# yukw777/EILEV

Measured on AMD Instinct MI355X. Metric: clips/sec (8-frame, 16 in-context) encode+generate, eilev-blip2-opt-2.7b, higher is better.
Workload: dtype bf16

## Files before the change

### eilev_amd/csrc/gemm_common.h

```cpp
#pragma once
#include "common.h"
#ifndef EILEV_ST_AUX
#define EILEV_ST_AUX 2
#endif
#include <type_traits>
#include <utility>

namespace {


constexpr int BK = 64;

__device__ __forceinline__ int swz(int row, int c) { return (c ^ ((row >> 1) & 7)) << 4; }

template <class F, int... I>
__device__ __forceinline__ void static_for_impl(F &&f, std::integer_sequence<int, I...>) {
    (f(std::integral_constant<int, I>{}), ...);
}
template <int N, class F>
__device__ __forceinline__ void static_for(F &&f) {
    static_for_impl(f, std::make_integer_sequence<int, N>{});
}

__device__ __forceinline__ void tile_coords(const GemmArgs &g, int tiles_m, int tiles_n, int &tm, int &tn, int t = blockIdx.x) {
    const int nwg = tiles_m * tiles_n;
    const int xcd = t & 7, q = nwg >> 3, r = nwg & 7;
    t = (xcd < r ? xcd * (q + 1) : r * (q + 1) + (xcd - r) * q) + (t >> 3);
    if (g.dbg & DBG_GEMM_ROW_MAJOR_TILES) {
        tm = t / tiles_n;
        tn = t % tiles_n;
        return;
    }
    const int gsel = (g.dbg >> DBG_GEMM_GROUP_SHIFT) & 3;
    const int GROUP_M = gsel == 1 ? 4 : gsel == 2 ? 8 : gsel == 3 ? 16 : (tiles_n <= 8 ? 4 : 8);
    const int width = GROUP_M * tiles_n, group = t / width, first = group * GROUP_M;
    const int gsz = min(tiles_m - first, GROUP_M), in = t - group * width;
    tm = first + in % gsz;
    tn = in / gsz;
}

template <int WM, int WN, int EPI, int IBEG = 0, int IEND = WM / 32, int LN = 0, bool FASTG = false>
__device__ __forceinline__ void gemm_epilogue(const GemmArgs &g, f32x16 (&acc)[WM / 32][WN / 32], char *smem, int m0, int n0,
                                              int wm, int wn, int wid, int lane) {
    constexpr int TN = WN / 32;
    constexpr int RS = WN * 2 + 8;
    constexpr int ROWS = (IEND - IBEG) * 32;
    const int l31 = lane & 31, hi = lane >> 5;
    const int wrow0 = m0 + wm * WM, wcol0 = n0 + wn * WN;
    if (g.out_f32) {
#pragma unroll
        for (int i = IBEG; i < IEND; ++i) {
            const int row = wrow0 + i * 32 + l31;
#pragma unroll
            for (int j = 0; j < TN; ++j)
#pragma unroll
                for (int q = 0; q < 4; ++q) {
                    const int col = wcol0 + j * 32 + q * 8 + hi * 4;
                    if (row < g.M && col < g.N && !((g.dbg & DBG_GEMM_ROW0_STORES) && row > 0)) {
                        float *dst = reinterpret_cast<float *>(g.C) + (int64_t)row * g.ldc + col;
#pragma unroll
                        for (int e = 0; e < 4; ++e) {
                            float v = acc[i][j][q * 4 + e];
                            if (g.ascale) v *= g.ascale[row];
                            if (g.wscale && col + e < g.N) v *= g.wscale[col + e];
                            if (g.bias) v += (float)g.bias[col + e];
                            if (col + e < g.scale_cols) v *= g.scale;
                            if (EPI == 1) v = gelu_erf(v);
                            else if (EPI == 2) v = fmaxf(v, 0.0f);
                            if (g.resid) v += (float)g.resid[(int64_t)row * g.ldr + col + e];
                            if (col + e < g.N) {
                                if (g.k_slice > 0) atomicAdd(dst + e, v);
                                else dst[e] = v;
                            }
                        }
                    }
                }
        }
        return;
    }
    if (g.dbg & DBG_GEMM_NO_EPILOGUE) {
        float keep = 0.0f;
#pragma unroll
        for (int i = IBEG; i < IEND; ++i)
#pragma unroll
            for (int j = 0; j < TN; ++j) keep += acc[i][j][0] + acc[i][j][7] + acc[i][j][15];
        if (keep == 123.456f) reinterpret_cast<float *>(g.C)[0] = keep;
        return;
    }
    float st1[LN == 2 ? IEND - IBEG : 1], st2[LN == 2 ? IEND - IBEG : 1];
    if constexpr (LN == 2) {
#pragma unroll
        for (int i = 0; i < IEND - IBEG; ++i) st1[i] = st2[i] = 0.0f;
    }
    char *reg = smem + wid * (ROWS * RS);
    const int wrow1 = wrow0 + IBEG * 32;
    const int srow = lane >> 3, schunk = lane & 7;
    const bool patch = g.patch_group > 0;
    const bool interior = wrow1 + ROWS <= g.M && wcol0 + WN <= g.N && !patch && !(g.dbg & DBG_GEMM_ROW0_STORES);
    const bool has_res = g.resid != nullptr;
    const bool has_scale = g.scale_cols > 0;
    if (has_res) {
        if (interior) {
            const bf16 *rp = g.resid + (int64_t)(wrow1 + srow) * g.ldr + wcol0 + schunk * 8;
            char *dp = reg + srow * RS + schunk * 16;
#pragma unroll 4
            for (int it = 0; it < ROWS / 8; ++it) {
                const bf16x8 v = *reinterpret_cast<const bf16x8 *>(rp);
                bf16x4 *d = reinterpret_cast<bf16x4 *>(dp);
                d[0] = (bf16x4){v[0], v[1], v[2], v[3]};
                d[1] = (bf16x4){v[4], v[5], v[6], v[7]};
                rp += 8 * g.ldr;
                dp += 8 * RS;
            }
        } else {
#pragma unroll 2
            for (int it = 0; it < ROWS / 8; ++it) {
                const int lr = it * 8 + srow, row = wrow1 + lr, col = wcol0 + schunk * 8;
                bf16x8 v = zero8();
                if (row < g.M && col < g.N) {
                    const int64_t rrow = patch ? 1 + (row % g.patch_group) : row;
                    v = *reinterpret_cast<const bf16x8 *>(g.resid + rrow * g.ldr + col);
                }
                bf16x4 *d = reinterpret_cast<bf16x4 *>(reg + lr * RS + schunk * 16);
                d[0] = (bf16x4){v[0], v[1], v[2], v[3]};
                d[1] = (bf16x4){v[4], v[5], v[6], v[7]};
            }
        }
    }
#pragma unroll
    for (int j = 0; j < TN; ++j) {
#pragma unroll
        for (int q = 0; q < 4; ++q) {
            const int lc = j * 32 + q * 8 + hi * 4, col = wcol0 + lc;
            float bv[4] = {0.f, 0.f, 0.f, 0.f};
            if (g.bias && col < g.N) {
                const bf16x4 b4 = *reinterpret_cast<const bf16x4 *>(g.bias + col);
#pragma unroll
                for (int e = 0; e < 4; ++e) bv[e] = (float)b4[e];
            }
            float sc[4] = {1.f, 1.f, 1.f, 1.f};
            if (has_scale) {
#pragma unroll
                for (int e = 0; e < 4; ++e) sc[e] = (col + e) < g.scale_cols ? g.scale : 1.0f;
            }
            char *cp = reg + l31 * RS + lc * 2;
            constexpr int NI = IEND - IBEG;
            float v[NI][4];
            if (g.wscale) {
#pragma unroll
                for (int e = 0; e < 4; ++e) {
                    const float ws = col + e < g.N ? g.wscale[col + e] : 1.0f;
#pragma unroll
                    for (int i = 0; i < NI; ++i) acc[IBEG + i][j][q * 4 + e] *= ws;
                }
            }
            if (g.ascale) {
#pragma unroll
                for (int i = 0; i < NI; ++i) {
                    const int row = wrow0 + (IBEG + i) * 32 + l31;
                    const float as = row < g.M ? g.ascale[row] : 1.0f;
#pragma unroll
                    for (int e = 0; e < 4; ++e) acc[IBEG + i][j][q * 4 + e] *= as;
                }
            }
            if (LN == 1) {
#pragma unroll
                for (int i = 0; i < NI; ++i) {
                    const int row = wrow0 + (IBEG + i) * 32 + l31;
                    const float la = row < g.M ? g.ln_rows[2 * (int64_t)row] : 1.0f;
#pragma unroll
                    for (int e = 0; e < 4; ++e) acc[IBEG + i][j][q * 4 + e] *= la;
                }
            }
#pragma unroll
            for (int i = 0; i < NI; ++i)
#pragma unroll
                for (int e = 0; e < 4; ++e) {
                    v[i][e] = acc[IBEG + i][j][q * 4 + e] + bv[e];
                    if (has_scale) v[i][e] *= sc[e];
                    if (EPI == 2) v[i][e] = fmaxf(v[i][e], 0.0f);
                }
            if (EPI == 1) {
                f32x2 x[2 * NI];
#pragma unroll
                for (int i = 0; i < NI; ++i) {
                    x[2 * i] = (f32x2){v[i][0], v[i][1]};
                    x[2 * i + 1] = (f32x2){v[i][2], v[i][3]};
                }
                if constexpr (FASTG) {
                    float y[4 * NI];
#pragma unroll
                    for (int i = 0; i < 2 * NI; ++i) { y[2 * i] = x[i].x; y[2 * i + 1] = x[i].y; }
                    gelu_erf_n<4 * NI>(y);
#pragma unroll
                    for (int i = 0; i < 2 * NI; ++i) x[i] = (f32x2){y[2 * i], y[2 * i + 1]};
                } else gelu_erf_pk<2 * NI>(x);
#pragma unroll
                for (int i = 0; i < NI; ++i) {
                    v[i][0] = x[2 * i].x; v[i][1] = x[2 * i].y; v[i][2] = x[2 * i + 1].x; v[i][3] = x[2 * i + 1].y;
                }
            }
#pragma unroll
            for (int i = 0; i < NI; ++i) {
                bf16x4 *cell = reinterpret_cast<bf16x4 *>(cp + i * 32 * RS);
                if (has_res) {
                    const bf16x4 r4 = *cell;
#pragma unroll
                    for (int e = 0; e < 4; ++e) v[i][e] += (float)r4[e];
                }
                if (LN == 2) {
#pragma unroll
                    for (int e = 0; e < 4; ++e)
                        if (col + e < g.N) {
                            st1[LN == 2 ? i : 0] += v[i][e];
                            st2[LN == 2 ? i : 0] = fmaf(v[i][e], v[i][e], st2[LN == 2 ? i : 0]);
                        }
                }
                *cell = (bf16x4){(bf16)v[i][0], (bf16)v[i][1], (bf16)v[i][2], (bf16)v[i][3]};
            }
        }
    }
    if (LN == 2 && wcol0 < g.N) {
        static_assert(WN == 64, "one statistics slot per 64 columns");
#pragma unroll
        for (int i = 0; i < IEND - IBEG; ++i) {
            const float t1 = st1[LN == 2 ? i : 0] + __shfl_xor(st1[LN == 2 ? i : 0], 32), t2 = st2[LN == 2 ? i : 0] + __shfl_xor(st2[LN == 2 ? i : 0], 32);
            const int row = wrow0 + (IBEG + i) * 32 + l31;
            if (hi == 0 && row < g.M)
                *reinterpret_cast<float2 *>(g.stat_out + ((int64_t)(wcol0 >> 6) * g.stat_ld + row) * 2) = make_float2(t1, t2);
        }
    }
    if (g.dbg & DBG_GEMM_NO_STORES) return;
    if (interior) {
        bf16 *dp = reinterpret_cast<bf16 *>(g.C) + (int64_t)(wrow1 + srow) * g.ldc + wcol0 + schunk * 8;
        const char *sp0 = reg + srow * RS + schunk * 16;
#pragma unroll 4
        for (int it = 0; it < ROWS / 8; ++it) {
            const bf16x4 *sp = reinterpret_cast<const bf16x4 *>(sp0);
            const bf16x4 lo = sp[0], hi4 = sp[1];
            *reinterpret_cast<bf16x8 *>(dp) = (bf16x8){lo[0], lo[1], lo[2], lo[3], hi4[0], hi4[1], hi4[2], hi4[3]};
            dp += 8 * g.ldc;
            sp0 += 8 * RS;
        }
        return;
    }
#pragma unroll 2
    for (int it = 0; it < ROWS / 8; ++it) {
        const int lr = it * 8 + srow, row = wrow1 + lr, col = wcol0 + schunk * 8;
        if (row < g.M && col < g.N && !((g.dbg & DBG_GEMM_ROW0_STORES) && row > 0)) {
            const bf16x4 *sp = reinterpret_cast<const bf16x4 *>(reg + lr * RS + schunk * 16);
            const bf16x4 lo = sp[0], hi4 = sp[1];
            int64_t orow = row;
            if (patch) {
                const int f = row / g.patch_group;
                orow = row + f + 1;
            }
            bf16 *dst = reinterpret_cast<bf16 *>(g.C) + orow * g.ldc + col;
            if (col + 8 <= g.N) {
                *reinterpret_cast<bf16x8 *>(dst) = (bf16x8){lo[0], lo[1], lo[2], lo[3], hi4[0], hi4[1], hi4[2], hi4[3]};
            } else {
#pragma unroll
                for (int e = 0; e < 4; ++e) {
                    if (col + e < g.N) dst[e] = lo[e];
                    if (col + 4 + e < g.N) dst[4 + e] = hi4[e];
                }
            }
        }
    }
}

typedef __attribute__((address_space(3))) void lds_void;


}
```

### eilev_amd/csrc/gemm_pp4.h

```cpp
#pragma once
#include "gemm_common.h"

namespace {

#ifndef EILEV_PP4_DEEP
#define EILEV_PP4_DEEP 1
#endif
template <int EPI, bool F8 = false, int LN = 0, int M16K = 0, bool A3 = false>
__global__ __launch_bounds__(512, 2) void gemm_pp4_kernel(const GemmArgs g) {
    constexpr bool M16 = M16K != 0, HT16 = M16K == 2;
    static_assert(!M16 || !F8, "16 x 16 form: bf16 instances");
    constexpr int BM = 256, BN = 256, NWM = 2, NWN = 4, NW = 8;
    constexpr int WM = BM / NWM, WN = BN / NWN, TM = WM / 32, TN = WN / 32;
    constexpr int STEP = (BM + BN) * 128;
    constexpr int PC = 8;
    static_assert(!A3 || M16, "A3: lean epilogues only");
    constexpr int STG0 = A3 ? 2 * BM * 128 : 2 * STEP;

    extern __shared__ __attribute__((aligned(16))) char smem[];
    auto a_slot = [&](int st) { return smem + (A3 ? (st % 3) * (BM * 128) : (st & 1) * STEP); };
    auto w_slot = [&](int st) { return smem + (A3 ? 3 * (BM * 128) + (st & 1) * (BN * 128) : (st & 1) * STEP + BM * 128); };
    const int tiles_m = (g.M + BM - 1) / BM, tiles_n = (g.N + BN - 1) / BN, ntiles = tiles_m * tiles_n;
    const int tid = threadIdx.x, lane = tid & 63;
    const int wid = __builtin_amdgcn_readfirstlane(tid >> 6);
    const int wm = wid / NWN, wn = wid % NWN;
    const int l31 = lane & 31, hi = lane >> 5;
    const int l15 = lane & 15, g4 = lane >> 4;
    constexpr int TM16 = WM / 16, TN16 = WN / 16;
    const int ns = g.K / 64;
    const bool late = wid >= NW / 2;
    const int prow = lane >> 3, pslot = lane & 7;

    __amdgpu_buffer_rsrc_t ra = __builtin_amdgcn_make_buffer_rsrc((void *)g.A, 0, 0x7fffffff, 0x00020000);
    const __amdgpu_buffer_rsrc_t rw = __builtin_amdgcn_make_buffer_rsrc((void *)g.W, 0, 0x7fffffff, 0x00020000);
    unsigned po[PC];
    const int pw = late ? wid - NW / 2 : wid;
    auto set_tile = [&](int t, int &m0, int &n0) {
        int tm_i, tn_i;
        tile_coords(g, tiles_m, tiles_n, tm_i, tn_i, t);
        m0 = tm_i * BM;
        n0 = tn_i * BN;
        {
#ifdef EILEV_PP4_PROBE_A0
            const uint64_t base = (uint64_t)(g.A);
#else
            const uint64_t base = (uint64_t)(g.A + (int64_t)m0 * g.lda);
#endif
            const uint64_t ub = ((uint64_t)(unsigned)__builtin_amdgcn_readfirstlane((int)(base >> 32)) << 32) |
                                (unsigned)__builtin_amdgcn_readfirstlane((int)(unsigned)base);
            ra = __builtin_amdgcn_make_buffer_rsrc((void *)ub, 0, 0x7fffffff, 0x00020000);
        }
#pragma unroll
        for (int i = 0; i < PC; ++i) {
            const int row = (pw * PC + i) * 8 + prow;
            const unsigned sw = (unsigned)((pslot ^ ((row >> 1) & 7)) << 4);
            if (!late) {
                int gr = m0 + row;
                gr = gr < g.M ? gr : g.M - 1;
                po[i] = (unsigned)(gr - m0) * (unsigned)(g.lda * 2) + sw;
            } else {
                int gr = n0 + row;
                gr = gr < g.N ? gr : g.N - 1;
                po[i] = (unsigned)gr * (unsigned)(g.ldw * 2) + sw;
            }
        }
    };
    auto stage_step = [&](int st, bool mine = true, int part = 0) {
        char *sd = (late ? w_slot(st) : a_slot(st)) + (pw * PC) * 1024;
        if (!mine) return;
#ifndef EILEV_PP4_PROBE_SKIP
#define EILEV_PP4_PROBE_SKIP 0
#endif
        constexpr int PCE = (EILEV_PP4_PROBE_SKIP & 4) ? 0 : (EILEV_PP4_PROBE_SKIP & 1) ? PC / 2 : PC;
        constexpr int PCL = (EILEV_PP4_PROBE_SKIP & 8) ? 0 : (EILEV_PP4_PROBE_SKIP & 2) ? PC / 2 : PC;
        if (late) {
#pragma unroll
            for (int i = 0; i < PCL; ++i)
                if (part == 0 || (part == 1) == (i < PC / 2)) __builtin_amdgcn_raw_ptr_buffer_load_lds(rw, (lds_void *)(sd + i * 1024), 16, po[i], st * 128, 0, 0);
        } else {
#pragma unroll
            for (int i = 0; i < PCE; ++i)
                if (part == 0 || (part == 1) == (i < PC / 2)) __builtin_amdgcn_raw_ptr_buffer_load_lds(ra, (lds_void *)(sd + i * 1024), 16, po[i], st * 128, 0, 0);
        }
    };
    f32x16 acc[M16 ? 1 : TM][M16 ? 1 : TN];
    bf16x8 af[2][TM], bfr[2][TN];
    typedef __attribute__((ext_vector_type(4))) float f32x4_t;
    f32x4_t acc16[M16 ? TM16 : 1][M16 ? TN16 : 1];
    auto read_half = [&](int st, int h) {
        const char *sa = a_slot(st) + (wm * WM) * 128;
        const char *sb = w_slot(st) + (wn * WN) * 128;
        if constexpr (M16) {
            const int kc = h * 4 + g4;
#pragma unroll
            for (int j = 0; j < TN16; ++j) {
                const int row = j * 16 + l15;
                bfr[j >> 1][j & 1] = *reinterpret_cast<const bf16x8 *>(sb + row * 128 + swz(row, kc));
            }
#pragma unroll
            for (int i = 0; i < TM16; ++i) {
                const int row = i * 16 + l15;
                af[i >> 2][i & 3] = *reinterpret_cast<const bf16x8 *>(sa + row * 128 + swz(row, kc));
            }
            return;
        }
#pragma unroll
        for (int k2 = 0; k2 < 2; ++k2) {
            const int kc = h * 4 + k2 * 2 + hi;
#pragma unroll
            for (int j = 0; j < TN; ++j) {
                const int row = j * 32 + l31;
                bfr[k2][j] = *reinterpret_cast<const bf16x8 *>(sb + row * 128 + swz(row, kc));
            }
#pragma unroll
            for (int i = 0; i < TM; ++i) {
                const int row = i * 32 + l31;
                af[k2][i] = *reinterpret_cast<const bf16x8 *>(sa + row * 128 + swz(row, kc));
            }
        }
    };
    typedef int i32x8_t __attribute__((ext_vector_type(8)));
    struct Pair16 { bf16x8 lo, hi; };
    auto cat32 = [](const bf16x8 &lo, const bf16x8 &hi2) { return __builtin_bit_cast(i32x8_t, Pair16{lo, hi2}); };
    auto mma_half = [&]() {
        __builtin_amdgcn_s_setprio(1);
        if constexpr (F8) {
#pragma unroll
            for (int i = 0; i < TM; ++i)
#pragma unroll
                for (int j = 0; j < TN; ++j)
                    acc[i][j] = __builtin_amdgcn_mfma_scale_f32_32x32x64_f8f6f4(cat32(bfr[0][j], bfr[1][j]), cat32(af[0][i], af[1][i]), acc[i][j],
                                                                               0, 0, 0, 0, 0, 0);
        } else if constexpr (M16) {
#pragma unroll
            for (int i = 0; i < TM16; ++i)
#pragma unroll
                for (int j = 0; j < TN16; ++j)
                    acc16[i][j] = __builtin_amdgcn_mfma_f32_16x16x32_bf16(bfr[j >> 1][j & 1], af[i >> 2][i & 3], acc16[i][j], 0, 0, 0);
        } else {
#pragma unroll
            for (int k2 = 0; k2 < 2; ++k2)
#pragma unroll
                for (int i = 0; i < TM; ++i)
#pragma unroll
                    for (int j = 0; j < TN; ++j)
                        acc[i][j] = __builtin_amdgcn_mfma_f32_32x32x16_bf16(bfr[k2][j], af[k2][i], acc[i][j], 0, 0, 0);
        }
        __builtin_amdgcn_s_setprio(0);
    };
    const int hm = wm * 2 + (wn >> 1), hn = wn & 1;
    auto read_half_ht = [&](int st, int h) {
        const char *sa = a_slot(st) + (hm * 64) * 128;
        const char *sb = w_slot(st) + (hn * 64) * 128;
        if constexpr (M16) {
            const int kc = h * 4 + g4;
#pragma unroll
            for (int j = 0; j < 4; ++j) {
                const int row = j * 16 + l15;
                bfr[j >> 1][j & 1] = *reinterpret_cast<const bf16x8 *>(sb + row * 128 + swz(row, kc));
            }
#pragma unroll
            for (int i = 0; i < 4; ++i) {
                const int row = i * 16 + l15;
                af[0][i] = *reinterpret_cast<const bf16x8 *>(sa + row * 128 + swz(row, kc));
            }
            return;
        }
#pragma unroll
        for (int k2 = 0; k2 < 2; ++k2) {
            const int kc = h * 4 + k2 * 2 + hi;
#pragma unroll
            for (int j = 0; j < 2; ++j) {
                const int row = j * 32 + l31;
                bfr[k2][j] = *reinterpret_cast<const bf16x8 *>(sb + row * 128 + swz(row, kc));
            }
#pragma unroll
            for (int i = 0; i < 2; ++i) {
                const int row = i * 32 + l31;
                af[k2][i] = *reinterpret_cast<const bf16x8 *>(sa + row * 128 + swz(row, kc));
            }
        }
    };
    auto mma_half_ht = [&]() {
        __builtin_amdgcn_s_setprio(1);
        if constexpr (F8) {
#pragma unroll
            for (int i = 0; i < 2; ++i)
#pragma unroll
                for (int j = 0; j < 2; ++j)
                    acc[i][j] = __builtin_amdgcn_mfma_scale_f32_32x32x64_f8f6f4(cat32(bfr[0][j], bfr[1][j]), cat32(af[0][i], af[1][i]), acc[i][j],
                                                                               0, 0, 0, 0, 0, 0);
        } else if constexpr (M16) {
#pragma unroll
            for (int i = 0; i < 4; ++i)
#pragma unroll
                for (int j = 0; j < 4; ++j)
                    acc16[i][j] = __builtin_amdgcn_mfma_f32_16x16x32_bf16(bfr[j >> 1][j & 1], af[0][i], acc16[i][j], 0, 0, 0);
        } else {
#pragma unroll
            for (int k2 = 0; k2 < 2; ++k2)
#pragma unroll
                for (int i = 0; i < 2; ++i)
#pragma unroll
                    for (int j = 0; j < 2; ++j)
                        acc[i][j] = __builtin_amdgcn_mfma_f32_32x32x16_bf16(bfr[k2][j], af[k2][i], acc[i][j], 0, 0, 0);
        }
        __builtin_amdgcn_s_setprio(0);
    };
    char *const stg = smem + STG0 + wid * 4096;
    const unsigned stg_sw = (unsigned)(STG0 + wid * 4096 + l31 * 128 + hi * 8) ^ (unsigned)((l31 & 7) << 4);
    const unsigned stg_sw16 = (unsigned)(STG0 + wid * 4096 + l15 * 128 + (g4 & 1) * 8) ^ (unsigned)((((g4 >> 1) ^ (l15 & 7)) << 4));
    const int srow = lane >> 3, schunk = lane & 7;
    auto is_lean = [&](int n0_) {
        return !(n0_ + 128 >= g.N && !(g.dbg & DBG_GEMM_NO_HALF_TILES)) && n0_ + BN <= g.N && !g.out_f32 && g.patch_group == 0 && g.scale_cols == 0 && !g.wscale && !g.ascale &&
               !(g.dbg & (DBG_GEMM_NO_EPILOGUE | DBG_GEMM_NO_STORES | DBG_GEMM_ROW0_STORES)) && !(g.dbg & DBG_GEMM_PP4_NO_PRESTAGE);
    };
    float ln_rs[LN == 1 ? (M16 ? TM16 : TM) : 1];
    auto lean_epilogue = [&](int cm0, int cn0, auto res_c, auto ht_c) {
        constexpr bool RES = decltype(res_c)::value;
        constexpr bool HTE = decltype(ht_c)::value;
        constexpr int NU = HTE ? 2 : TM;
        const int roff = HTE ? hm * 64 : wm * WM, coff = HTE ? hn * 64 : wn * WN;
        if constexpr (M16K == 1) {
            if (cn0 + coff >= g.N) return;
        }
        constexpr bool LNC = LN == 1 && !RES, LNP = LN == 2 && RES;
        typedef __attribute__((ext_vector_type(4))) unsigned u32x4_t;
        const int r0 = cm0 + roff;
        const int rows = g.M - r0 < 0 ? 0 : (g.M - r0 < NU * 32 ? g.M - r0 : NU * 32);
        auto uniform_rsrc = [&](const void *ptr, int bytes) {
            const uint64_t base = (uint64_t)ptr;
            const uint64_t ub = ((uint64_t)(unsigned)__builtin_amdgcn_readfirstlane((int)(base >> 32)) << 32) |
                                (unsigned)__builtin_amdgcn_readfirstlane((int)(unsigned)base);
            return __builtin_amdgcn_make_buffer_rsrc((void *)ub, 0, __builtin_amdgcn_readfirstlane(bytes), 0x00020000);
        };
        const __amdgpu_buffer_rsrc_t rc = uniform_rsrc(reinterpret_cast<bf16 *>(g.C) + (int64_t)r0 * g.ldc + cn0 + coff, rows * (int)(g.ldc * 2));
        const __amdgpu_buffer_rsrc_t rr = uniform_rsrc(RES ? g.resid + (int64_t)r0 * g.ldr + cn0 + coff : g.A, RES ? rows * (int)(g.ldr * 2) : 0);
        const unsigned st_voff = (unsigned)srow * (unsigned)(g.ldc * 2) + schunk * 16, rs_voff = (unsigned)srow * (unsigned)(g.ldr * 2) + schunk * 16;
#ifndef EILEV_HM_AUX
#define EILEV_HM_AUX EILEV_ST_AUX
#endif
        constexpr bool HMI = LN == 1 && !RES && EPI == 0 && M16K == 1;
        const bool hm = HMI && g.hm_tok != 0;
        __amdgpu_buffer_rsrc_t rch = rc;
        unsigned hm_off = 0, hm_off_w = 0;
        int hm_str2 = 0, hm_t = 0;
        if constexpr (HMI) {
            if (hm) {
                const int TOK = g.hm_tok, HD = g.hm_hd, NH = g.hm_heads, D3 = g.N / 3;
                const int n0 = cn0 + coff;
                const int plane = __builtin_amdgcn_readfirstlane(n0 / D3), rr = n0 - plane * D3;
                int2 ent;
                if (rr < NH * 64) {
                    ent.x = (plane * NH + (rr >> 6)) * TOK * HD + schunk * 8;
                    ent.y = 64;
                } else {
                    const int cph = (HD - 64) >> 3, jb = ((rr - NH * 64) >> 3) + schunk, hh = jb / cph;
                    ent.x = (plane * NH + hh) * TOK * HD + TOK * 64 + (jb - hh * cph) * 8;
                    ent.y = HD - 64;
                }
                const int fw = __builtin_amdgcn_readfirstlane(r0 / TOK);
                const int m0 = r0 + srow, f0 = m0 / TOK;
                hm_t = m0 - f0 * TOK;
                hm_str2 = __builtin_amdgcn_readfirstlane(ent.y * 2);
                hm_off = (unsigned)(((f0 - fw) * TOK * g.N + ent.x + hm_t * ent.y) * 2);
                hm_off_w = hm_off + (unsigned)(TOK * g.N * 2) - (unsigned)(TOK * hm_str2);
                const int64_t left = ((int64_t)g.M / TOK - fw) * TOK * g.N * 2;
                rch = uniform_rsrc(reinterpret_cast<bf16 *>(g.C) + (int64_t)fw * TOK * g.N, (int)(unsigned)(left < 0xfffffff0ll ? left : 0xfffffff0ll));
            }
        }
        u32x4_t rv[4];
        auto res_load = [&](int u) {
#pragma unroll
            for (int it = 0; it < 4; ++it) rv[it] = __builtin_amdgcn_raw_buffer_load_b128(rr, rs_voff, (u * 32 + it * 8) * (int)(g.ldr * 2), 0);
        };
        if constexpr (RES) res_load(0);
        bf16x4 biasr[M16 ? 1 : TN][4];
        bf16x4 biasr16[M16 ? TN16 : 1];
        if constexpr (M16) {
#pragma unroll
            for (int j = 0; j < TN16; ++j) {
                if (g.bias) biasr16[j] = *reinterpret_cast<const bf16x4 *>(g.bias + cn0 + coff + j * 16 + g4 * 4);
                else biasr16[j] = (bf16x4){(bf16)0.f, (bf16)0.f, (bf16)0.f, (bf16)0.f};
            }
        } else {
#pragma unroll
        for (int j = 0; j < TN; ++j)
#pragma unroll
            for (int q = 0; q < 4; ++q) {
                if (g.bias) biasr[j][q] = *reinterpret_cast<const bf16x4 *>(g.bias + cn0 + wn * WN + j * 32 + q * 8 + hi * 4);
                else biasr[j][q] = (bf16x4){(bf16)0.f, (bf16)0.f, (bf16)0.f, (bf16)0.f};
            }
        }
        typedef __attribute__((ext_vector_type(2))) float f32x2_t;
        __amdgpu_buffer_rsrc_t rst = rr;
        if constexpr (LNP) rst = uniform_rsrc(g.stat_out + ((int64_t)((cn0 + coff) >> 6) * g.stat_ld + r0) * 2, rows * 8);
        static_for<NU>([&](auto u_c) {
            constexpr int U = decltype(u_c)::value;
            float st1 = 0.0f, st2 = 0.0f;
            bf16x4 rcell[M16 ? 2 : TN][4];
            if constexpr (RES) {
#pragma unroll
                for (int it = 0; it < 4; ++it) {
                    const int row = it * 8 + srow;
                    *reinterpret_cast<u32x4_t *>(stg + row * 128 + ((schunk ^ (row & 7)) << 4)) = rv[it];
                }
                if constexpr (U + 1 < NU) res_load(U + 1);
                if constexpr (M16) {
#pragma unroll
                    for (int ib = 0; ib < 2; ++ib)
#pragma unroll
                        for (int j = 0; j < TN16; ++j) {
                            unsigned ca;
                            asm volatile("v_xor_b32 %0, %1, %2" : "=v"(ca) : "n"(((j * 2) << 4) | (ib << 11)), "v"(stg_sw16));
                            rcell[ib][j] = *reinterpret_cast<const bf16x4 *>(smem + ca);
                        }
                } else {
#pragma unroll
                for (int j = 0; j < TN; ++j)
#pragma unroll
                    for (int q = 0; q < 4; ++q) {
                        unsigned ca;
                        asm volatile("v_xor_b32 %0, %1, %2" : "=v"(ca) : "n"((j * 4 + q) << 4), "v"(stg_sw));
                        rcell[j][q] = *reinterpret_cast<const bf16x4 *>(smem + ca);
                    }
                }
            }
            float st16[2][2] = {{0.0f, 0.0f}, {0.0f, 0.0f}};
            if constexpr (M16) {
#pragma unroll
                for (int ib = 0; ib < 2; ++ib)
#pragma unroll
                    for (int j = 0; j < TN16; ++j) {
                        float v[4];
                        if constexpr (LNC) {
#pragma unroll
                            for (int e = 0; e < 4; ++e) v[e] = fmaf(acc16[2 * U + ib][j][e], ln_rs[2 * U + ib], (float)biasr16[j][e]);
                        } else {
#pragma unroll
                            for (int e = 0; e < 4; ++e) v[e] = acc16[2 * U + ib][j][e] + (float)biasr16[j][e];
                        }
                        if constexpr (LN == 0 && EPI == 0 && !RES) {
                            if (cn0 + coff + j * 16 < g.scale_cols) {
#pragma unroll
                                for (int e = 0; e < 4; ++e) v[e] *= g.scale;
                            }
                        }
                        if constexpr (EPI == 2) {
#pragma unroll
                            for (int e = 0; e < 4; ++e) v[e] = fmaxf(v[e], 0.0f);
                        }
                        if constexpr (EPI == 1) gelu_erf_n<4>(v);
                        if constexpr (RES) {
#pragma unroll
                            for (int e = 0; e < 4; ++e) v[e] += (float)rcell[ib][j][e];
                        }
                        if constexpr (LNP) {
#pragma unroll
                            for (int e = 0; e < 4; ++e) {
                                st16[ib][0] += v[e];
                                st16[ib][1] = fmaf(v[e], v[e], st16[ib][1]);
                            }
                        }
                        unsigned ca;
                        asm volatile("v_xor_b32 %0, %1, %2" : "=v"(ca) : "n"(((j * 2) << 4) | (ib << 11)), "v"(stg_sw16));
                        *reinterpret_cast<bf16x4 *>(smem + ca) = (bf16x4){(bf16)v[0], (bf16)v[1], (bf16)v[2], (bf16)v[3]};
                    }
            } else {
#pragma unroll
            for (int j = 0; j < TN; ++j)
#pragma unroll
                for (int q = 0; q < 4; ++q) {
                    float v[4];
                    if constexpr (LNC) {
#pragma unroll
                        for (int e = 0; e < 4; ++e) v[e] = fmaf(acc[U][j][q * 4 + e], ln_rs[U], (float)biasr[j][q][e]);
                    } else {
#pragma unroll
                        for (int e = 0; e < 4; ++e) v[e] = acc[U][j][q * 4 + e] + (float)biasr[j][q][e];
                    }
                    if constexpr (EPI == 2) {
#pragma unroll
                        for (int e = 0; e < 4; ++e) v[e] = fmaxf(v[e], 0.0f);
                    }
                    if constexpr (EPI == 1) gelu_erf_n<4>(v);
                    if constexpr (RES) {
#pragma unroll
                        for (int e = 0; e < 4; ++e) v[e] += (float)rcell[j][q][e];
                    }
                    if constexpr (LNP) {
#pragma unroll
                        for (int e = 0; e < 4; ++e) {
                            st1 += v[e];
                            st2 = fmaf(v[e], v[e], st2);
                        }
                    }
                    unsigned ca;
                    asm volatile("v_xor_b32 %0, %1, %2" : "=v"(ca) : "n"((j * 4 + q) << 4), "v"(stg_sw));
                    *reinterpret_cast<bf16x4 *>(smem + ca) = (bf16x4){(bf16)v[0], (bf16)v[1], (bf16)v[2], (bf16)v[3]};
                }
            }
            if constexpr (LNP && M16) {
                typedef __attribute__((ext_vector_type(2))) unsigned u32x2_t;
#pragma unroll
                for (int ib = 0; ib < 2; ++ib) {
                    float a1 = st16[ib][0], a2 = st16[ib][1];
                    a1 += __shfl_xor(a1, 16); a2 += __shfl_xor(a2, 16);
                    a1 += __shfl_xor(a1, 32); a2 += __shfl_xor(a2, 32);
                    const f32x2_t t = (f32x2_t){a1, a2};
                    if (g4 == 0) __builtin_amdgcn_raw_buffer_store_b64(__builtin_bit_cast(u32x2_t, t), rst, (U * 32 + ib * 16 + l15) * 8, 0, 0);
                }
            } else if constexpr (LNP) {
                typedef __attribute__((ext_vector_type(2))) unsigned u32x2_t;
                const f32x2_t t = (f32x2_t){st1 + __shfl_xor(st1, 32), st2 + __shfl_xor(st2, 32)};
                if (hi == 0) __builtin_amdgcn_raw_buffer_store_b64(__builtin_bit_cast(u32x2_t, t), rst, (U * 32 + l31) * 8, 0, 0);
            }
            __builtin_amdgcn_sched_barrier(0);
            bf16x8 erb[2];
#pragma unroll
            for (int h2 = 0; h2 < 2; ++h2) {
#pragma unroll
                for (int b = 0; b < 2; ++b) {
                    const int row = (h2 * 2 + b) * 8 + srow;
                    erb[b] = *reinterpret_cast<const bf16x8 *>(stg + row * 128 + ((schunk ^ (row & 7)) << 4));
                }
                if (hm) {
                    if constexpr (HMI) {
#pragma unroll
                        for (int b = 0; b < 2; ++b) {
                            const int RO = U * 32 + (h2 * 2 + b) * 8;
                            const unsigned vo = hm_t + RO >= g.hm_tok ? hm_off_w : hm_off;
                            __builtin_amdgcn_raw_buffer_store_b128(__builtin_bit_cast(u32x4_t, erb[b]), rch, vo, RO * hm_str2, EILEV_HM_AUX);
                        }
                    }
                } else {
#pragma unroll
                for (int b = 0; b < 2; ++b)
                    __builtin_amdgcn_raw_buffer_store_b128(__builtin_bit_cast(u32x4_t, erb[b]), rc, st_voff, (U * 32 + (h2 * 2 + b) * 8) * (int)(g.ldc * 2), EILEV_ST_AUX);
                }
            }
            asm volatile("s_nop 1" ::: "memory");
            __builtin_amdgcn_sched_barrier(0);
        });
    };
#define PP_WAIT_LGKM0() __builtin_amdgcn_s_waitcnt(0xC07F)
#define PP_WAIT_LGKM0_VM0() __builtin_amdgcn_s_waitcnt(0x0070)
#define PP_WAIT_VM0() __builtin_amdgcn_s_waitcnt(0x0F70)
#define PP_BARRIER()                       \
    do {                                   \
        __builtin_amdgcn_sched_barrier(0); \
        __builtin_amdgcn_s_barrier();      \
        __builtin_amdgcn_sched_barrier(0); \
    } while (0)

    int t = blockIdx.x, m0, n0;
    if (t >= ntiles) return;
    set_tile(t, m0, n0);
    auto w_piece_mine = [&](int n0_) { return !(n0_ + 128 >= g.N && !(g.dbg & DBG_GEMM_NO_HALF_TILES)) || wid < NW / 2 + 2; };
    stage_step(0, w_piece_mine(n0));
    bool pre1 = ns > 1 && (A3 || !(g.dbg & DBG_GEMM_PP4_NO_PRESTAGE));
    if (pre1) stage_step(1, w_piece_mine(n0));
    bool lean_cur = M16 || is_lean(n0);
    float ln_nm[LN == 1 ? (M16 ? TM16 : TM) : 1], ln_cl[LN == 1 ? (M16 ? TN16 : TN) : 1];
    auto ln_fetch = [&](int m0_, int n0_) {
        if constexpr (LN == 1 && M16) {
            const bool ht = HT16 && n0_ + 128 >= g.N;
            const int mb = m0_ + (ht ? hm * 64 : wm * WM) + l15, nb = n0_ + (ht ? hn * 64 : wn * WN) + l15;
            const __amdgpu_buffer_rsrc_t rl = __builtin_amdgcn_make_buffer_rsrc((void *)g.ln_rows, 0, g.M * 8, 0x00020000);
            const __amdgpu_buffer_rsrc_t rcs = __builtin_amdgcn_make_buffer_rsrc((void *)g.ln_csum, 0, g.N * 4, 0x00020000);
#pragma unroll
            for (int i = 0; i < TM16; ++i) ln_nm[i] = __builtin_bit_cast(float, __builtin_amdgcn_raw_buffer_load_b32(rl, (mb + i * 16) * 8 + 4, 0, 0));
#pragma unroll
            for (int j = 0; j < TN16; ++j) ln_cl[j] = __builtin_bit_cast(float, __builtin_amdgcn_raw_buffer_load_b32(rcs, (nb + j * 16) * 4, 0, 0));
        } else if constexpr (LN == 1) {
            const bool ht = n0_ + 128 >= g.N && !(g.dbg & DBG_GEMM_NO_HALF_TILES);
            const int mb = m0_ + (ht ? hm * 64 : wm * WM) + l31, nb = n0_ + (ht ? hn * 64 : wn * WN) + l31;
            const __amdgpu_buffer_rsrc_t rl = __builtin_amdgcn_make_buffer_rsrc((void *)g.ln_rows, 0, g.M * 8, 0x00020000);
            const __amdgpu_buffer_rsrc_t rcs = __builtin_amdgcn_make_buffer_rsrc((void *)g.ln_csum, 0, g.N * 4, 0x00020000);
#pragma unroll
            for (int i = 0; i < TM; ++i) ln_nm[i] = __builtin_bit_cast(float, __builtin_amdgcn_raw_buffer_load_b32(rl, (mb + i * 32) * 8 + 4, 0, 0));
#pragma unroll
            for (int j = 0; j < TN; ++j) ln_cl[j] = __builtin_bit_cast(float, __builtin_amdgcn_raw_buffer_load_b32(rcs, (nb + j * 32) * 4, 0, 0));
        }
    };
    ln_fetch(m0, n0);
    int trace_i = 0;
    const bool tracer = g.trace != nullptr && (wid == 0 || wid == NW / 2) && lane == 0;
#ifdef EILEV_PP4_ITRACE
#define ITR(k)                                                                                                              \
    do {                                                                                                                    \
        if (st == EILEV_PP4_ITRACE && tracer) *reinterpret_cast<volatile unsigned long long *>(stg + (k) * 8) = __builtin_amdgcn_s_memtime(); \
    } while (0)
#else
#define ITR(k) do { } while (0)
#endif
    auto stamp = [&](int k, bool core = false) {
#ifdef EILEV_PP4_ITRACE
        return;
#endif
        if (tracer && trace_i < g.trace_tiles)
            g.trace[(((size_t)blockIdx.x * 2 + (late ? 1 : 0)) * g.trace_tiles + trace_i) * 8 + k] =
                core ? __builtin_amdgcn_s_memtime() : __builtin_amdgcn_s_memrealtime();
    };
    for (; t < ntiles; t += gridDim.x) {
        stamp(0);
        stamp(5, true);
        typedef __attribute__((ext_vector_type(4))) short s16x4_t;
        s16x4_t ln_a1[LN == 1 ? (M16 ? TM16 : TM) : 1], ln_w1[LN == 1 ? (M16 ? TN16 : TN) : 1];
        auto acc_prep = [&]() {
            if constexpr (LN == 1 && M16) {
                const bf16 z = (bf16)0.0f;
#pragma unroll
                for (int i = 0; i < TM16; ++i) {
                    const float m = g4 ? 0.0f : ln_nm[i];
                    const bf16 mh = (bf16)m, ml = (bf16)(m - (float)mh);
                    ln_a1[i] = __builtin_bit_cast(s16x4_t, (bf16x4){mh, mh, ml, z});
                }
#pragma unroll
                for (int j = 0; j < TN16; ++j) {
                    const float c = g4 ? 0.0f : ln_cl[j];
                    const bf16 ch = (bf16)c, cl = (bf16)(c - (float)ch);
                    ln_w1[j] = __builtin_bit_cast(s16x4_t, (bf16x4){ch, cl, ch, z});
                }
            } else if constexpr (LN == 1) {
                const bf16 z = (bf16)0.0f;
#pragma unroll
                for (int i = 0; i < TM; ++i) {
                    const float m = hi ? 0.0f : ln_nm[i];
                    const bf16 mh = (bf16)m, ml = (bf16)(m - (float)mh);
                    ln_a1[i] = __builtin_bit_cast(s16x4_t, (bf16x4){mh, mh, ml, z});
                }
#pragma unroll
                for (int j = 0; j < TN; ++j) {
                    const float c = hi ? 0.0f : ln_cl[j];
                    const bf16 ch = (bf16)c, cl = (bf16)(c - (float)ch);
                    ln_w1[j] = __builtin_bit_cast(s16x4_t, (bf16x4){ch, cl, ch, z});
                }
            }
        };
        auto acc_init = [&]() {
            if constexpr (M16) {
                const f32x4_t zero4 = (f32x4_t){0.0f, 0.0f, 0.0f, 0.0f};
#pragma unroll
                for (int i = 0; i < TM16; ++i)
#pragma unroll
                    for (int j = 0; j < TN16; ++j) {
                        if constexpr (LN == 1) acc16[i][j] = __builtin_amdgcn_mfma_f32_16x16x16bf16_1k(ln_w1[j], ln_a1[i], zero4, 0, 0, 0);
                        else acc16[i][j] = zero4;
                    }
            } else if constexpr (LN == 1) {
                f32x16 zero;
#pragma unroll
                for (int r = 0; r < 16; ++r) zero[r] = 0.0f;
#pragma unroll
                for (int i = 0; i < TM; ++i)
#pragma unroll
                    for (int j = 0; j < TN; ++j) acc[i][j] = __builtin_amdgcn_mfma_f32_32x32x8bf16_1k(ln_w1[j], ln_a1[i], zero, 0, 0, 0);
            } else {
#pragma unroll
                for (int i = 0; i < TM; ++i)
#pragma unroll
                    for (int j = 0; j < TN; ++j)
#pragma unroll
                        for (int r = 0; r < 16; ++r) acc[i][j][r] = 0.0f;
            }
        };
        if constexpr (LN != 1) acc_init();
        asm volatile("s_waitcnt vmcnt(0)" ::: "memory");
        PP_BARRIER();
        if (late) PP_BARRIER();
        stamp(1);
        const int nsd = (g.dbg & DBG_GEMM_ONE_KSTEP) ? 1 : ns;
        const bool half_tile = n0 + 128 >= g.N && !(g.dbg & DBG_GEMM_NO_HALF_TILES);
        auto kstep = [&](int st, auto first_c, auto ht_c) {
            constexpr bool FIRST = decltype(first_c)::value;
            constexpr bool HT = decltype(ht_c)::value;
            const bool w_mine = !HT || wid < NW / 2 + 2;
            ITR(0);
            if constexpr (HT) read_half_ht(st, 0); else read_half(st, 0);
#if EILEV_PP4_DEEP
#ifndef EILEV_PP4_SPLIT
#define EILEV_PP4_SPLIT 3
#endif
#ifndef EILEV_PP4_SPLIT_QKV
#define EILEV_PP4_SPLIT_QKV 0
#endif
            constexpr bool SPLIT_OK = !HT && (EILEV_PP4_SPLIT_QKV || !(LN == 1 && EPI == 0));
            constexpr bool SPLIT_E = (EILEV_PP4_SPLIT & 1) && SPLIT_OK, SPLIT_L = (EILEV_PP4_SPLIT & 2) && SPLIT_OK;
            if (!late) {
                if constexpr (A3) {
                    if (st + 2 < ns) stage_step(st + 2, w_mine, SPLIT_E ? 1 : 0);
                } else if (st + 1 < ns && !(FIRST && pre1)) stage_step(st + 1, w_mine, SPLIT_E ? 1 : 0);
            } else if (FIRST && !pre1 && ns > 1) stage_step(1, w_mine);
            else if (SPLIT_L && !FIRST && st + 1 < ns) stage_step(st + 1, w_mine, 2);
#else
            if (st + 1 < ns && !(FIRST && pre1)) stage_step(st + 1, w_mine);
#endif
            if constexpr (FIRST && LN == 1) acc_prep();
            PP_WAIT_LGKM0();
            ITR(1);
            PP_BARRIER();
            ITR(2);
            if constexpr (FIRST && LN == 1) acc_init();
            if constexpr (HT) mma_half_ht(); else mma_half();
            ITR(3);
            PP_BARRIER();
            ITR(4);
            if constexpr (HT) read_half_ht(st, 1); else read_half(st, 1);
#if EILEV_PP4_DEEP
            PP_WAIT_LGKM0();
            if (late) {
                PP_WAIT_VM0();
                if constexpr (!HT) if (st + 2 < ns) stage_step(st + 2, w_mine, SPLIT_L ? 1 : 0);
            } else if (A3) {
                if (SPLIT_E && st + 2 < ns) stage_step(st + 2, w_mine, 2);
            } else if (SPLIT_E && st + 1 < ns && !(FIRST && pre1)) stage_step(st + 1, w_mine, 2);
            ITR(5);
            PP_BARRIER();
            ITR(6);
            if constexpr (HT) {
                if (late && st + 2 < ns) stage_step(st + 2, w_mine);
                mma_half_ht();
            } else mma_half();
            __builtin_amdgcn_sched_barrier(0);
            if constexpr (A3) {
                if (!late) {
                    if (st + 2 < ns) asm volatile("s_waitcnt vmcnt(8)" ::: "memory");
                    else asm volatile("s_waitcnt vmcnt(0)" ::: "memory");
                }
            } else if (!late) asm volatile("s_waitcnt vmcnt(0)" ::: "memory");
            ITR(7);
            PP_BARRIER();
#else
            PP_WAIT_LGKM0_VM0();
            PP_BARRIER();
            if constexpr (HT) mma_half_ht(); else mma_half();
            PP_BARRIER();
#endif
        };
        if (half_tile && M16K != 1) {
            if constexpr (M16K != 1) {
                kstep(0, std::true_type{}, std::true_type{});
                for (int st = 1; st < nsd; ++st) kstep(st, std::false_type{}, std::true_type{});
            }
        } else {
            kstep(0, std::true_type{}, std::false_type{});
            for (int st = 1; st < nsd; ++st) kstep(st, std::false_type{}, std::false_type{});
        }
        stamp(2);
#ifdef EILEV_PP4_ITRACE
        if (tracer && trace_i < g.trace_tiles) {
#pragma unroll
            for (int k = 0; k < 8; ++k)
                g.trace[(((size_t)blockIdx.x * 2 + (late ? 1 : 0)) * g.trace_tiles + trace_i) * 8 + k] = *reinterpret_cast<volatile unsigned long long *>(stg + k * 8);
        }
#endif
        if (!late) PP_BARRIER();
        if constexpr (LN == 1) {
            const __amdgpu_buffer_rsrc_t rl = __builtin_amdgcn_make_buffer_rsrc((void *)g.ln_rows, 0, g.M * 8, 0x00020000);
            if constexpr (M16) {
#pragma unroll
                for (int i = 0; i < TM16; ++i) ln_rs[i] = __builtin_bit_cast(float, __builtin_amdgcn_raw_buffer_load_b32(rl, (m0 + ((HT16 && half_tile) ? hm * 64 : wm * WM) + i * 16 + l15) * 8, 0, 0));
            } else {
#pragma unroll
            for (int u = 0; u < TM; ++u) ln_rs[u] = __builtin_bit_cast(float, __builtin_amdgcn_raw_buffer_load_b32(rl, (m0 + wm * WM + u * 32 + l31) * 8, 0, 0));
            }
        }
        const int cm0 = m0, cn0 = n0, tn = t + gridDim.x;
        const bool lean = lean_cur;
        pre1 = false;
        lean_cur = false;
        if (tn < ntiles) {
            set_tile(tn, m0, n0);
            stage_step(0, w_piece_mine(n0));
            pre1 = lean && ns > 1;
            if (pre1) stage_step(1, w_piece_mine(n0));
            lean_cur = M16 || is_lean(n0);
            ln_fetch(m0, n0);
        }
        stamp(3);
        if (HT16 && half_tile) {
            if constexpr (HT16) {
                if constexpr (LN == 1) lean_epilogue(cm0, cn0, std::false_type{}, std::true_type{});
                else if constexpr (LN == 2) lean_epilogue(cm0, cn0, std::true_type{}, std::true_type{});
                else if (g.resid != nullptr) lean_epilogue(cm0, cn0, std::true_type{}, std::true_type{});
                else lean_epilogue(cm0, cn0, std::false_type{}, std::true_type{});
            }
        } else if (lean || M16) {
            if constexpr (LN == 1) lean_epilogue(cm0, cn0, std::false_type{}, std::false_type{});
            else if constexpr (LN == 2) lean_epilogue(cm0, cn0, std::true_type{}, std::false_type{});
            else if (g.resid != nullptr) lean_epilogue(cm0, cn0, std::true_type{}, std::false_type{});
            else lean_epilogue(cm0, cn0, std::false_type{}, std::false_type{});
        } else if constexpr (!M16) {
            if (half_tile) {
                gemm_epilogue<64, 64, EPI, 0, 2, LN, true>(g, reinterpret_cast<f32x16(&)[2][2]>(acc), smem + STEP, cm0, cn0, hm, hn, wid, lane);
            } else {
                gemm_epilogue<WM, WN, EPI, 0, TM / 2, LN, true>(g, acc, smem + STEP, cm0, cn0, wm, wn, wid, lane);
                gemm_epilogue<WM, WN, EPI, TM / 2, TM, LN, true>(g, acc, smem + STEP, cm0, cn0, wm, wn, wid, lane);
            }
        }
        stamp(4);
        stamp(6, true);
        ++trace_i;
    }
#undef PP_BARRIER
}

constexpr int PP4_SMEM = 2 * 65536 + 8 * 4096;

}
```

Measured before the change: 224.6.

## Use 384x128 tall tiles for the ragged last N column in half-tile GEMM

When N leaves a 128-wide remainder, the half-tile HT16 GEMM now covers that last column with 384x128 tiles instead of 256x128 half tiles. A new tile scheduler interleaves these tall tiles with the full 256x256 tiles in groups. The staging loads are redistributed so all eight waves fill the 384-row A slice and the 128-row W slice. The aim is to fix the poor MFMA utilisation and load imbalance of the half tiles and to cut the number of tail workgroups. In exchange the tile-to-workgroup mapping and LDS layout become more complex, and each wave carries more accumulators in the tall case.

```diff
diff --git a/eilev_amd/csrc/gemm_common.h b/eilev_amd/csrc/gemm_common.h
--- a/eilev_amd/csrc/gemm_common.h
+++ b/eilev_amd/csrc/gemm_common.h
@@ -37,6 +37,23 @@
     const int gsz = min(tiles_m - first, GROUP_M), in = t - group * width;
     tm = first + in % gsz;
     tn = in / gsz;
+}
+
+__host__ __device__ __forceinline__ int tall_ntiles(int M, int N) { return ((M + 255) / 256) * (N / 256) + (M + 383) / 384; }
+__device__ __forceinline__ void tile_coords_tall(const GemmArgs &g, int &m0, int &n0, int t = blockIdx.x) {
+    const int tiles_m = (g.M + 255) / 256, tn_full = g.N / 256, nwg = tall_ntiles(g.M, g.N);
+    const int xcd = t & 7, q = nwg >> 3, r = nwg & 7;
+    t = (xcd < r ? xcd * (q + 1) : r * (q + 1) + (xcd - r) * q) + (t >> 3);
+    const int gfull = 4 * tn_full + 3, period = 3 * gfull - 1, sup = t / period, rem = t - sup * period;
+    const int gi = rem >= 2 * gfull ? 2 : rem >= gfull ? 1 : 0, group = sup * 3 + gi, first = group * 4, in = rem - gi * gfull;
+    const int gsz = min(tiles_m - first, 4), whole = gsz * tn_full;
+    if (in < whole) {
+        m0 = (first + in % gsz) * 256;
+        n0 = (in / gsz) * 256;
+    } else {
+        m0 = ((8 * group + 2) / 3 + in - whole) * 384;
+        n0 = tn_full * 256;
+    }
 }
 
 template <int WM, int WN, int EPI, int IBEG = 0, int IEND = WM / 32, int LN = 0, bool FASTG = false>
diff --git a/eilev_amd/csrc/gemm_pp4.h b/eilev_amd/csrc/gemm_pp4.h
--- a/eilev_amd/csrc/gemm_pp4.h
+++ b/eilev_amd/csrc/gemm_pp4.h
@@ -9,6 +9,9 @@
 template <int EPI, bool F8 = false, int LN = 0, int M16K = 0, bool A3 = false>
 __global__ __launch_bounds__(512, 2) void gemm_pp4_kernel(const GemmArgs g) {
     constexpr bool M16 = M16K != 0, HT16 = M16K == 2;
+    constexpr bool TALL = HT16 && !A3;
+    constexpr int TALL_BM = 384;
+    constexpr int HT_WM = TALL ? TALL_BM / 4 : 64, HT_TM16 = HT_WM / 16;
     static_assert(!M16 || !F8, "16 x 16 form: bf16 instances");
     constexpr int BM = 256, BN = 256, NWM = 2, NWN = 4, NW = 8;
     constexpr int WM = BM / NWM, WN = BN / NWN, TM = WM / 32, TN = WN / 32;
@@ -20,7 +23,8 @@
     extern __shared__ __attribute__((aligned(16))) char smem[];
     auto a_slot = [&](int st) { return smem + (A3 ? (st % 3) * (BM * 128) : (st & 1) * STEP); };
     auto w_slot = [&](int st) { return smem + (A3 ? 3 * (BM * 128) + (st & 1) * (BN * 128) : (st & 1) * STEP + BM * 128); };
-    const int tiles_m = (g.M + BM - 1) / BM, tiles_n = (g.N + BN - 1) / BN, ntiles = tiles_m * tiles_n;
+    const bool tall_n = TALL && (g.N & 255) == 128;
+    const int tiles_m = (g.M + BM - 1) / BM, tiles_n = (g.N + BN - 1) / BN, ntiles = tall_n ? tall_ntiles(g.M, g.N) : tiles_m * tiles_n;
     const int tid = threadIdx.x, lane = tid & 63;
     const int wid = __builtin_amdgcn_readfirstlane(tid >> 6);
     const int wm = wid / NWN, wn = wid % NWN;
@@ -35,11 +39,25 @@
     const __amdgpu_buffer_rsrc_t rw = __builtin_amdgcn_make_buffer_rsrc((void *)g.W, 0, 0x7fffffff, 0x00020000);
     unsigned po[PC];
     const int pw = late ? wid - NW / 2 : wid;
+    bool src_a = !late;
+    bool src_a_hi = !late;
+    int d_lo = wid * (PC * 1024), d_hi = wid * (PC * 1024) + (PC / 2) * 1024;
     auto set_tile = [&](int t, int &m0, int &n0) {
-        int tm_i, tn_i;
-        tile_coords(g, tiles_m, tiles_n, tm_i, tn_i, t);
-        m0 = tm_i * BM;
-        n0 = tn_i * BN;
+        if (tall_n) {
+            if constexpr (TALL) tile_coords_tall(g, m0, n0, t);
+        } else {
+            int tm_i, tn_i;
+            tile_coords(g, tiles_m, tiles_n, tm_i, tn_i, t);
+            m0 = tm_i * BM;
+            n0 = tn_i * BN;
+        }
+        const bool tt = TALL && n0 + 128 >= g.N;
+        src_a = !late || tt;
+        src_a_hi = tt ? late : !late;
+        if constexpr (TALL) {
+            d_lo = tt ? (pw * HT_WM + (late ? 0 : 64)) * 128 : wid * (PC * 1024);
+            d_hi = tt ? (late ? d_lo + (PC / 2) * 1024 : (TALL_BM + pw * 32) * 128) : d_lo + (PC / 2) * 1024;
+        }
         {
 #ifdef EILEV_PP4_PROBE_A0
             const uint64_t base = (uint64_t)(g.A);
@@ -52,9 +70,9 @@
         }
 #pragma unroll
         for (int i = 0; i < PC; ++i) {
-            const int row = (pw * PC + i) * 8 + prow;
+            const int row = (!tt ? (pw * PC + i) * 8 : late ? pw * HT_WM + i * 8 : i < PC / 2 ? pw * HT_WM + 64 + i * 8 : pw * 32 + (i - PC / 2) * 8) + prow;
             const unsigned sw = (unsigned)((pslot ^ ((row >> 1) & 7)) << 4);
-            if (!late) {
+            if (i < PC / 2 ? src_a : src_a_hi) {
                 int gr = m0 + row;
                 gr = gr < g.M ? gr : g.M - 1;
                 po[i] = (unsigned)(gr - m0) * (unsigned)(g.lda * 2) + sw;
@@ -73,7 +91,20 @@
 #endif
         constexpr int PCE = (EILEV_PP4_PROBE_SKIP & 4) ? 0 : (EILEV_PP4_PROBE_SKIP & 1) ? PC / 2 : PC;
         constexpr int PCL = (EILEV_PP4_PROBE_SKIP & 8) ? 0 : (EILEV_PP4_PROBE_SKIP & 2) ? PC / 2 : PC;
-        if (late) {
+        if constexpr (TALL) {
+            char *sb2 = smem + (st & 1) * STEP;
+            auto issue4 = [&](int i0, bool from_a, char *dst) {
+                if (from_a) {
+#pragma unroll
+                    for (int i = 0; i < PC / 2; ++i) __builtin_amdgcn_raw_ptr_buffer_load_lds(ra, (lds_void *)(dst + i * 1024), 16, po[i0 + i], st * 128, 0, 0);
+                } else {
+#pragma unroll
+                    for (int i = 0; i < PC / 2; ++i) __builtin_amdgcn_raw_ptr_buffer_load_lds(rw, (lds_void *)(dst + i * 1024), 16, po[i0 + i], st * 128, 0, 0);
+                }
+            };
+            if (part != 2) issue4(0, src_a, sb2 + d_lo);
+            if (part != 1) issue4(PC / 2, src_a_hi, sb2 + d_hi);
+        } else if (late) {
 #pragma unroll
             for (int i = 0; i < PCL; ++i)
                 if (part == 0 || (part == 1) == (i < PC / 2)) __builtin_amdgcn_raw_ptr_buffer_load_lds(rw, (lds_void *)(sd + i * 1024), 16, po[i], st * 128, 0, 0);
@@ -148,10 +179,10 @@
         }
         __builtin_amdgcn_s_setprio(0);
     };
-    const int hm = wm * 2 + (wn >> 1), hn = wn & 1;
+    const int hm = TALL ? wid & 3 : wm * 2 + (wn >> 1), hn = TALL ? wid >> 2 : wn & 1;
     auto read_half_ht = [&](int st, int h) {
-        const char *sa = a_slot(st) + (hm * 64) * 128;
-        const char *sb = w_slot(st) + (hn * 64) * 128;
+        const char *sa = a_slot(st) + (hm * HT_WM) * 128;
+        const char *sb = (TALL ? a_slot(st) + TALL_BM * 128 : w_slot(st)) + (hn * 64) * 128;
         if constexpr (M16) {
             const int kc = h * 4 + g4;
 #pragma unroll
@@ -160,9 +191,9 @@
                 bfr[j >> 1][j & 1] = *reinterpret_cast<const bf16x8 *>(sb + row * 128 + swz(row, kc));
             }
 #pragma unroll
-            for (int i = 0; i < 4; ++i) {
+            for (int i = 0; i < HT_TM16; ++i) {
                 const int row = i * 16 + l15;
-                af[0][i] = *reinterpret_cast<const bf16x8 *>(sa + row * 128 + swz(row, kc));
+                af[i >> 2][i & 3] = *reinterpret_cast<const bf16x8 *>(sa + row * 128 + swz(row, kc));
             }
             return;
         }
@@ -192,10 +223,10 @@
                                                                                0, 0, 0, 0, 0, 0);
         } else if constexpr (M16) {
 #pragma unroll
-            for (int i = 0; i < 4; ++i)
+            for (int i = 0; i < HT_TM16; ++i)
 #pragma unroll
                 for (int j = 0; j < 4; ++j)
-                    acc16[i][j] = __builtin_amdgcn_mfma_f32_16x16x32_bf16(bfr[j >> 1][j & 1], af[0][i], acc16[i][j], 0, 0, 0);
+                    acc16[i][j] = __builtin_amdgcn_mfma_f32_16x16x32_bf16(bfr[j >> 1][j & 1], af[i >> 2][i & 3], acc16[i][j], 0, 0, 0);
         } else {
 #pragma unroll
             for (int k2 = 0; k2 < 2; ++k2)
@@ -219,8 +250,8 @@
     auto lean_epilogue = [&](int cm0, int cn0, auto res_c, auto ht_c) {
         constexpr bool RES = decltype(res_c)::value;
         constexpr bool HTE = decltype(ht_c)::value;
-        constexpr int NU = HTE ? 2 : TM;
-        const int roff = HTE ? hm * 64 : wm * WM, coff = HTE ? hn * 64 : wn * WN;
+        constexpr int NU = HTE ? HT_WM / 32 : TM;
+        const int roff = HTE ? hm * HT_WM : wm * WM, coff = HTE ? hn * 64 : wn * WN;
         if constexpr (M16K == 1) {
             if (cn0 + coff >= g.N) return;
         }
@@ -456,7 +487,7 @@
     int t = blockIdx.x, m0, n0;
     if (t >= ntiles) return;
     set_tile(t, m0, n0);
-    auto w_piece_mine = [&](int n0_) { return !(n0_ + 128 >= g.N && !(g.dbg & DBG_GEMM_NO_HALF_TILES)) || wid < NW / 2 + 2; };
+    auto w_piece_mine = [&](int n0_) { return TALL || !(n0_ + 128 >= g.N && !(g.dbg & DBG_GEMM_NO_HALF_TILES)) || wid < NW / 2 + 2; };
     stage_step(0, w_piece_mine(n0));
     bool pre1 = ns > 1 && (A3 || !(g.dbg & DBG_GEMM_PP4_NO_PRESTAGE));
     if (pre1) stage_step(1, w_piece_mine(n0));
@@ -465,7 +496,7 @@
     auto ln_fetch = [&](int m0_, int n0_) {
         if constexpr (LN == 1 && M16) {
             const bool ht = HT16 && n0_ + 128 >= g.N;
-            const int mb = m0_ + (ht ? hm * 64 : wm * WM) + l15, nb = n0_ + (ht ? hn * 64 : wn * WN) + l15;
+            const int mb = m0_ + (ht ? hm * HT_WM : wm * WM) + l15, nb = n0_ + (ht ? hn * 64 : wn * WN) + l15;
             const __amdgpu_buffer_rsrc_t rl = __builtin_amdgcn_make_buffer_rsrc((void *)g.ln_rows, 0, g.M * 8, 0x00020000);
             const __amdgpu_buffer_rsrc_t rcs = __builtin_amdgcn_make_buffer_rsrc((void *)g.ln_csum, 0, g.N * 4, 0x00020000);
 #pragma unroll
@@ -575,7 +606,7 @@
         auto kstep = [&](int st, auto first_c, auto ht_c) {
             constexpr bool FIRST = decltype(first_c)::value;
             constexpr bool HT = decltype(ht_c)::value;
-            const bool w_mine = !HT || wid < NW / 2 + 2;
+            const bool w_mine = !HT || TALL || wid < NW / 2 + 2;
             ITR(0);
             if constexpr (HT) read_half_ht(st, 0); else read_half(st, 0);
 #if EILEV_PP4_DEEP
@@ -585,7 +616,7 @@
 #ifndef EILEV_PP4_SPLIT_QKV
 #define EILEV_PP4_SPLIT_QKV 0
 #endif
-            constexpr bool SPLIT_OK = !HT && (EILEV_PP4_SPLIT_QKV || !(LN == 1 && EPI == 0));
+            constexpr bool SPLIT_OK = (!HT || TALL) && (EILEV_PP4_SPLIT_QKV || !(LN == 1 && EPI == 0));
             constexpr bool SPLIT_E = (EILEV_PP4_SPLIT & 1) && SPLIT_OK, SPLIT_L = (EILEV_PP4_SPLIT & 2) && SPLIT_OK;
             if (!late) {
                 if constexpr (A3) {
@@ -611,7 +642,7 @@
             PP_WAIT_LGKM0();
             if (late) {
                 PP_WAIT_VM0();
-                if constexpr (!HT) if (st + 2 < ns) stage_step(st + 2, w_mine, SPLIT_L ? 1 : 0);
+                if constexpr (!HT || TALL) if (st + 2 < ns) stage_step(st + 2, w_mine, SPLIT_L ? 1 : 0);
             } else if (A3) {
                 if (SPLIT_E && st + 2 < ns) stage_step(st + 2, w_mine, 2);
             } else if (SPLIT_E && st + 1 < ns && !(FIRST && pre1)) stage_step(st + 1, w_mine, 2);
@@ -619,7 +650,7 @@
             PP_BARRIER();
             ITR(6);
             if constexpr (HT) {
-                if (late && st + 2 < ns) stage_step(st + 2, w_mine);
+                if constexpr (!TALL) if (late && st + 2 < ns) stage_step(st + 2, w_mine);
                 mma_half_ht();
             } else mma_half();
             __builtin_amdgcn_sched_barrier(0);
@@ -660,7 +691,7 @@
             const __amdgpu_buffer_rsrc_t rl = __builtin_amdgcn_make_buffer_rsrc((void *)g.ln_rows, 0, g.M * 8, 0x00020000);
             if constexpr (M16) {
 #pragma unroll
-                for (int i = 0; i < TM16; ++i) ln_rs[i] = __builtin_bit_cast(float, __builtin_amdgcn_raw_buffer_load_b32(rl, (m0 + ((HT16 && half_tile) ? hm * 64 : wm * WM) + i * 16 + l15) * 8, 0, 0));
+                for (int i = 0; i < TM16; ++i) ln_rs[i] = __builtin_bit_cast(float, __builtin_amdgcn_raw_buffer_load_b32(rl, (m0 + ((HT16 && half_tile) ? hm * HT_WM : wm * WM) + i * 16 + l15) * 8, 0, 0));
             } else {
 #pragma unroll
             for (int u = 0; u < TM; ++u) ln_rs[u] = __builtin_bit_cast(float, __builtin_amdgcn_raw_buffer_load_b32(rl, (m0 + wm * WM + u * 32 + l31) * 8, 0, 0));
```

Measured after the change: 226.9, median of 6. 1.0% higher.
